# gercap/gr-ofdm_tools

Hardware: AMD Instinct MI355X
Metric: IQ Msamples/s Welch-PSD (4096-pt, 50% ovlp) (higher is better)
Workload: dtype f32; 1 GPU; C2: 2^28-sample complex64 stream, 4096-pt Hann Welch, 50% overlap, detrend constant, density; nfft=4096, noverlap=2048, window=hann, samples_per_gpu=268435456, segments_per_gpu=131071, parallelism=single GPU

## Files before the change

gr-ofdm_tools_amd/csrc/fft4096.hip.h:

```cpp
#pragma once
#include "fft_lds.hip.h"
#include "oth_internal.h"
#include "pinned_load.hip.h"
#include "twiddle16.hip.h"

static_assert(oth::kPilotProbes == 8, "load_pilot() (fft_lds.hip.h) adds eight probe means");

namespace oth {
namespace {

constexpr int T4 = 256;
constexpr int RS = 272;
constexpr int LDS_X = 16 * RS;
constexpr int LDS_RED = 16;
constexpr size_t LDS_BYTES = (LDS_X + LDS_RED) * sizeof(float2);

constexpr float C1 = 0.92387953251128674f;
constexpr float S1 = 0.38268343236508977f;
constexpr float RH = 0.70710678118654752f;

__device__ __forceinline__ float2 mul_w1(float2 a) { return make_float2(fmaf(a.x, C1, a.y * S1), fmaf(a.y, C1, -a.x * S1)); }
__device__ __forceinline__ float2 mul_w2(float2 a) { return make_float2((a.x + a.y) * RH, (a.y - a.x) * RH); }
__device__ __forceinline__ float2 mul_w3(float2 a) { return make_float2(fmaf(a.x, S1, a.y * C1), fmaf(a.y, S1, -a.x * C1)); }
__device__ __forceinline__ float2 mul_w4(float2 a) { return make_float2(a.y, -a.x); }
__device__ __forceinline__ float2 mul_w6(float2 a) { return make_float2((a.y - a.x) * RH, -(a.x + a.y) * RH); }
__device__ __forceinline__ float2 mul_w9(float2 a) { return make_float2(-fmaf(a.x, C1, a.y * S1), fmaf(a.x, S1, -a.y * C1)); }

constexpr float T1 = 0.41421356237309503f;

__device__ __forceinline__ void dft4_tail(float2 t0, float2 t1, float2 p1, float2 p3, float S, float2 &a0, float2 &a1,
                                          float2 &a2, float2 &a3) {
    const float2 q = cadd(p1, p3), r = csub(p1, p3);
    a0 = make_float2(fmaf(S, q.x, t0.x), fmaf(S, q.y, t0.y));
    a2 = make_float2(fmaf(-S, q.x, t0.x), fmaf(-S, q.y, t0.y));
    a1 = make_float2(fmaf(S, r.y, t1.x), fmaf(-S, r.x, t1.y));
    a3 = make_float2(fmaf(-S, r.y, t1.x), fmaf(S, r.x, t1.y));
}
template <bool PLAIN = false>
__device__ __forceinline__ void dft16_layer2(float2 (&v)[16]) {
  if constexpr (PLAIN) {
    v[5] = mul_w1(v[5]);
    v[9] = mul_w2(v[9]);
    v[13] = mul_w3(v[13]);
    v[6] = mul_w2(v[6]);
    v[10] = mul_w4(v[10]);
    v[14] = mul_w6(v[14]);
    v[7] = mul_w3(v[7]);
    v[11] = mul_w6(v[11]);
    v[15] = mul_w9(v[15]);
#pragma unroll
    for (int kl = 0; kl < 4; ++kl) dft4<false>(v[4 * kl], v[4 * kl + 1], v[4 * kl + 2], v[4 * kl + 3]);
  } else {
    dft4<false>(v[0], v[1], v[2], v[3]);
    {
        const float2 u1 = v[5], u2 = v[6], u3 = v[7];
        const float2 p1 = make_float2(fmaf(T1, u1.y, u1.x), fmaf(-T1, u1.x, u1.y));
        const float2 p2 = make_float2(u2.x + u2.y, u2.y - u2.x);
        const float2 p3 = make_float2(fmaf(T1, u3.x, u3.y), fmaf(T1, u3.y, -u3.x));
        const float2 t0 = make_float2(fmaf(RH, p2.x, v[4].x), fmaf(RH, p2.y, v[4].y));
        const float2 t1 = make_float2(fmaf(-RH, p2.x, v[4].x), fmaf(-RH, p2.y, v[4].y));
        dft4_tail(t0, t1, p1, p3, C1, v[4], v[5], v[6], v[7]);
    }
    {
        const float2 u1 = v[9], u2 = v[10], u3 = v[11];
        const float2 p1 = make_float2(u1.x + u1.y, u1.y - u1.x);
        const float2 p3 = make_float2(u3.y - u3.x, -u3.x - u3.y);
        const float2 t0 = make_float2(v[8].x + u2.y, v[8].y - u2.x);
        const float2 t1 = make_float2(v[8].x - u2.y, v[8].y + u2.x);
        dft4_tail(t0, t1, p1, p3, RH, v[8], v[9], v[10], v[11]);
    }
    {
        const float2 u1 = v[13], u2 = v[14], u3 = v[15];
        const float2 p1 = make_float2(fmaf(T1, u1.x, u1.y), fmaf(T1, u1.y, -u1.x));
        const float2 p2 = make_float2(u2.y - u2.x, -u2.x - u2.y);
        const float2 p3 = make_float2(fmaf(-T1, u3.y, -u3.x), fmaf(T1, u3.x, -u3.y));
        const float2 t0 = make_float2(fmaf(RH, p2.x, v[12].x), fmaf(RH, p2.y, v[12].y));
        const float2 t1 = make_float2(fmaf(-RH, p2.x, v[12].x), fmaf(-RH, p2.y, v[12].y));
        dft4_tail(t0, t1, p1, p3, C1, v[12], v[13], v[14], v[15]);
    }
  }
}

template <bool PLAIN = false>
__device__ __forceinline__ void dft16(float2 (&v)[16]) {
#pragma unroll
    for (int a0 = 0; a0 < 4; ++a0) dft4<false>(v[a0], v[a0 + 4], v[a0 + 8], v[a0 + 12]);
    dft16_layer2<PLAIN>(v);
}

template <bool PLAIN = false>
__device__ __forceinline__ void dft8(float2 (&v)[8]) {
    dft4<false>(v[0], v[2], v[4], v[6]);
    dft4<false>(v[1], v[3], v[5], v[7]);
    const float2 e0 = v[0], e1 = v[2], e2 = v[4], e3 = v[6];
    const float2 o0 = v[1], o2 = mul_w4(v[5]);
    if constexpr (PLAIN) {
        const float2 o1 = mul_w2(v[3]), o3 = mul_w6(v[7]);
        v[0] = cadd(e0, o0);
        v[4] = csub(e0, o0);
        v[1] = cadd(e1, o1);
        v[5] = csub(e1, o1);
        v[2] = cadd(e2, o2);
        v[6] = csub(e2, o2);
        v[3] = cadd(e3, o3);
        v[7] = csub(e3, o3);
        return;
    }
    const float2 p1 = make_float2(v[3].x + v[3].y, v[3].y - v[3].x);
    const float2 p3 = make_float2(v[7].y - v[7].x, -v[7].x - v[7].y);
    v[0] = cadd(e0, o0);
    v[4] = csub(e0, o0);
    v[1] = make_float2(fmaf(RH, p1.x, e1.x), fmaf(RH, p1.y, e1.y));
    v[5] = make_float2(fmaf(-RH, p1.x, e1.x), fmaf(-RH, p1.y, e1.y));
    v[2] = cadd(e2, o2);
    v[6] = csub(e2, o2);
    v[3] = make_float2(fmaf(RH, p3.x, e3.x), fmaf(RH, p3.y, e3.y));
    v[7] = make_float2(fmaf(-RH, p3.x, e3.x), fmaf(-RH, p3.y, e3.y));
}

typedef float lds_f4 __attribute__((ext_vector_type(4)));
template <bool WORD, bool SUMS> struct LdsCtl {
    const int *word_at;
    const float2 *sums_at;
    int word;
    lds_f4 s[2];
};
struct LdsNoMid {
    __device__ __forceinline__ void operator()() const {}
};

template <int STRIDE, class F, class M = LdsNoMid, bool WORD = false, bool SUMS = false>
__device__ __forceinline__ void dft16_from_lds(float2 (&v)[16], const float2 *base, F issued, M mid = M(),
                                               LdsCtl<WORD, SUMS> *ctl = nullptr) {
    const unsigned addr = (unsigned)(unsigned long long)base;
    double r[16];
    if constexpr (WORD) asm volatile("ds_read_b32 %0, %1" : "=v"(ctl->word) : "v"((unsigned)(unsigned long long)ctl->word_at));
    if constexpr (SUMS) {
        const unsigned sa = (unsigned)(unsigned long long)ctl->sums_at;
        asm volatile("ds_read_b128 %0, %1" : "=v"(ctl->s[0]) : "v"(sa));
        asm volatile("ds_read_b128 %0, %1 offset:16" : "=v"(ctl->s[1]) : "v"(sa));
    }
#define OTH_LDS_READ(i) asm volatile("ds_read_b64 %0, %1 offset:%2" : "=v"(r[i]) : "v"(addr), "n"(8 * STRIDE * (i)))
    OTH_LDS_READ(0); OTH_LDS_READ(4); OTH_LDS_READ(8); OTH_LDS_READ(12);
    OTH_LDS_READ(1); OTH_LDS_READ(5); OTH_LDS_READ(9); OTH_LDS_READ(13);
    OTH_LDS_READ(2); OTH_LDS_READ(6); OTH_LDS_READ(10); OTH_LDS_READ(14);
    OTH_LDS_READ(3); OTH_LDS_READ(7); OTH_LDS_READ(11); OTH_LDS_READ(15);
#undef OTH_LDS_READ
    issued();
#define OTH_LDS_WAIT(n, a, dep) \
    asm volatile("s_waitcnt lgkmcnt(" #n ")" : "+v"(r[a]), "+v"(r[a + 4]), "+v"(r[a + 8]), "+v"(r[a + 12]), "+v"(dep))
#pragma unroll
    for (int a0 = 0; a0 < 4; ++a0) {
        if (a0 == 0) {
            asm volatile("s_waitcnt lgkmcnt(12)" : "+v"(r[0]), "+v"(r[4]), "+v"(r[8]), "+v"(r[12]));
            if constexpr (SUMS) asm volatile("" : "+v"(ctl->s[0]), "+v"(ctl->s[1]));
        } else if (a0 == 1) OTH_LDS_WAIT(8, 1, v[0].x);
        else if (a0 == 2) OTH_LDS_WAIT(4, 2, v[1].x);
        else OTH_LDS_WAIT(0, 3, v[2].x);
#pragma unroll
        for (int j = 0; j < 4; ++j) v[a0 + 4 * j] = __builtin_bit_cast(float2, r[a0 + 4 * j]);
        dft4<false>(v[a0], v[a0 + 4], v[a0 + 8], v[a0 + 12]);
    }
#undef OTH_LDS_WAIT
    if constexpr (WORD) asm volatile("" : "+v"(ctl->word), "+v"(v[3].x), "+v"(v[15].y));
    mid();
    dft16_layer2(v);
}

__device__ __forceinline__ float2 load_once(const float2 *p) {
    typedef float f2 __attribute__((ext_vector_type(2)));
    const f2 r = __builtin_nontemporal_load(reinterpret_cast<const f2 *>(p));
    return make_float2(r.x, r.y);
}

__device__ __forceinline__ long long chunk_count(const WelchArgs &p) {
    const long long rest = p.nseg - p.nbig * p.chunk;
    return p.nbig + (rest + p.tail_chunk - 1) / p.tail_chunk;
}
__device__ __forceinline__ void chunk_range(const WelchArgs &p, long long c, long long &sb, long long &se) {
    if (c < p.nbig) {
        sb = c * p.chunk;
        se = sb + p.chunk;
    } else {
        sb = p.nbig * p.chunk + (c - p.nbig) * p.tail_chunk;
        se = sb + p.tail_chunk < p.nseg ? sb + p.tail_chunk : p.nseg;
    }
}

template <class I> __device__ __forceinline__ I chunk_count_of(I nseg, I nbig, int chunk, int tail_chunk) {
    const I rest = nseg - nbig * chunk;
    return nbig + (rest + tail_chunk - 1) / tail_chunk;
}
template <class I> __device__ __forceinline__ void chunk_range_of(I nseg, I nbig, int chunk, int tail_chunk, I c, I &sb, I &se) {
    if (c < nbig) {
        sb = c * chunk;
        se = sb + chunk;
    } else {
        sb = nbig * chunk + (c - nbig) * tail_chunk;
        se = sb + tail_chunk < nseg ? sb + tail_chunk : nseg;
    }
}

__device__ __forceinline__ void prio_latency() { __builtin_amdgcn_s_setprio(2); }
__device__ __forceinline__ void prio_compute() { __builtin_amdgcn_s_setprio(0); }

__device__ __forceinline__ void lds_barrier() { asm volatile("s_waitcnt lgkmcnt(0)\n\ts_barrier" ::: "memory"); }

__host__ __device__ constexpr int pow16_slot(int k) { return k - 5 - (k >> 2) + 1; }
template <int STRIDE, int NM>
__device__ __forceinline__ void scatter_pow16_stored(const float2 (&v)[16], float2 *out, float2 p1, float2 p2, float2 p3, float2 p4,
                                                     float2 p8, float2 p12, const float2 (&pm)[NM]) {
    float2 wj[4], wi[4];
    wj[1] = p1, wj[2] = p2, wj[3] = p3;
    wi[1] = p4, wi[2] = p8, wi[3] = p12;
#pragma unroll
    for (int i = 1; i < 4; ++i)
        if (pow16_slot(4 * i + 3) >= NM) asm volatile("" : "+v"(wi[i].x), "+v"(wi[i].y));
    out[0] = v[0];
#pragma unroll
    for (int k = 1; k < 16; ++k) {
        const int i = k >> 2, j = k & 3;
        float2 w;
        if (i == 0) w = wj[j];
        else if (j == 0) w = wi[i];
        else if (pow16_slot(k) < NM) w = pm[pow16_slot(k) < NM ? pow16_slot(k) : 0];
        else w = cmul(wi[i], wj[j]);
        out[STRIDE * k] = cmul(v[r16(k)], w);
    }
}

__device__ __forceinline__ void wave_lds_sync() {
    __builtin_amdgcn_fence(__ATOMIC_RELEASE, "wavefront");
    __builtin_amdgcn_wave_barrier();
    __builtin_amdgcn_fence(__ATOMIC_ACQUIRE, "wavefront");
}

template <int CTRL> __device__ __forceinline__ float dpp_add(float v) {
    const int x = __builtin_amdgcn_update_dpp(0, __float_as_int(v), CTRL, 0xF, 0xF, true);
    return v + __int_as_float(x);
}

__device__ __forceinline__ float wave_total(float v) {
    v = dpp_add<0xB1>(v);
    v = dpp_add<0x4E>(v);
    v = dpp_add<0x141>(v);
    v = dpp_add<0x140>(v);
    const int i = __float_as_int(v);
    return __int_as_float(__builtin_amdgcn_readlane(i, 0)) + __int_as_float(__builtin_amdgcn_readlane(i, 16)) +
           __int_as_float(__builtin_amdgcn_readlane(i, 32)) + __int_as_float(__builtin_amdgcn_readlane(i, 48));
}

__device__ __forceinline__ float wave_total_lane63(float v) {
    v = dpp_add<0xB1>(v);
    v = dpp_add<0x4E>(v);
    v = dpp_add<0x141>(v);
    v = dpp_add<0x140>(v);
    asm("s_nop 1\n\tv_add_f32_dpp %0, %0, %0 row_bcast:15 row_mask:0xa bank_mask:0xf" : "+v"(v));
    asm("s_nop 1\n\tv_add_f32_dpp %0, %0, %0 row_bcast:31 row_mask:0xc bank_mask:0xf" : "+v"(v));
    return v;
}

struct PilotProbes {
    float2 v[kPilotProbes];
};
__device__ __forceinline__ PilotProbes inline_pilot_load(const float2 *xb, long long nseg, int step, int t) {
    PilotProbes r;
#pragma unroll
    for (int k = 0; k < kPilotProbes; ++k) {
        const long long seg = ((nseg - 1) * k) / (kPilotProbes - 1);
        const float2 *src = xb + (size_t)__builtin_amdgcn_readfirstlane((int)seg) * (size_t)step + 512 * k;
        r.v[k] = src[(unsigned)t];
    }
    return r;
}
__device__ __forceinline__ void inline_pilot_store(const PilotProbes &r, int t, float2 *slot) {
#pragma unroll
    for (int k = 0; k < kPilotProbes; ++k) {
        const float2 s = make_float2(wave_total_lane63(r.v[k].x), wave_total_lane63(r.v[k].y));
        if ((t & 63) == 63) slot[4 * k + (t >> 6)] = s;
    }
}
__device__ __forceinline__ float2 inline_pilot_value(const float2 *slot) {
    float2 q[kPilotProbes];
#pragma unroll
    for (int k = 0; k < kPilotProbes; ++k) {
        const float2 a = cadd(slot[4 * k], slot[4 * k + 1]), b = cadd(slot[4 * k + 2], slot[4 * k + 3]);
        q[k] = make_float2((a.x + b.x) * (1.0f / 256.0f), (a.y + b.y) * (1.0f / 256.0f));
    }
    return pilot_of_probes(q);
}


}
}
```

gr-ofdm_tools_amd/csrc/welch4096ws.hip:

```cpp

#include <type_traits>
#include "fft4096.hip.h"
#include "launch.h"

namespace oth {
namespace {

constexpr int TWS = 512;
constexpr int WS_RED = 32;
constexpr int WS_CTRL = 16;
constexpr size_t WS_WIN_BYTES = 256 * 2 * sizeof(float4);
constexpr size_t WS_LDS_BYTES = (2 * LDS_X + WS_RED) * sizeof(float2) + WS_CTRL * sizeof(int) + WS_WIN_BYTES;

constexpr int WS_PAL = 2, WS_PAC = 0, WS_PAS = WS_PAL, WS_PBL = 2;
constexpr int WS_PBC = 1;

enum { ITEM_STOP = 0, ITEM_DATA = 1, ITEM_BUBBLE = 2 };

#ifndef OTH_WS_COMPL_POWERS
#define OTH_WS_COMPL_POWERS 13
#endif
constexpr int WS_COMPL_POWERS = OTH_WS_COMPL_POWERS;

template <bool DETREND, bool PILOT, bool COMPL>
__device__ __forceinline__ void welch4096ws_body(const WelchArgs &p) {
    static_assert(DETREND || !PILOT, "the pilot belongs to the detrend");
    extern __shared__ __attribute__((aligned(16))) unsigned char smem[];
    float2 *img = reinterpret_cast<float2 *>(smem);
    float2 *red = img + 2 * LDS_X;
    int *ctrl = reinterpret_cast<int *>(red + WS_RED);

    const int tid = threadIdx.x;
    const bool producer = tid < 256;
    const int t = tid & 255;
    const int hi = t >> 4, lo = t & 15;
    const int wave = t >> 6;
    const int wg = blockIdx.x, W = p.wg_per_stream, stream = blockIdx.y;
    const float2 *xb = p.x + (size_t)stream * p.stream_stride;
    const int sched = p.sched;
    const long long nchunks = sched ? chunk_count(p) : 1;

    const int w1 = hi * 17 + lo, r1 = hi * RS + lo, w2 = hi * RS + lo, r2 = hi * RS + lo * 17;

    if (producer) {
        float win[COMPL ? 1 : 8];
        float4 *wl = reinterpret_cast<float4 *>(ctrl + WS_CTRL) + t;
        constexpr int WROW = COMPL ? 0 : 8;
        if constexpr (!COMPL) {
#pragma unroll
            for (int a = 0; a < 8; ++a) win[a] = p.win[256 * a + t];
        }
        wl[0] = make_float4(p.win[256 * WROW + t], p.win[256 * (WROW + 1) + t], p.win[256 * (WROW + 2) + t], p.win[256 * (WROW + 3) + t]);
        wl[256] = make_float4(p.win[256 * (WROW + 4) + t], p.win[256 * (WROW + 5) + t], p.win[256 * (WROW + 6) + t],
                              p.win[256 * (WROW + 7) + t]);
        const float2 b1 = p.tw[t], b2 = p.tw[2 * t], b3 = p.tw[3 * t], b4 = p.tw[4 * t], b8 = p.tw[8 * t],
                     b12 = p.tw[(12 * t) & 4095];
        float2 bm[WS_COMPL_POWERS - 6 > 0 && COMPL ? WS_COMPL_POWERS - 6 : 1];
        if constexpr (COMPL) {
#pragma unroll
            for (int k = 0; k < WS_COMPL_POWERS - 6; ++k) bm[k] = p.tw[((5 + k + k / 3) * t) & 4095];
        }
        float2 kw[8], nxt[8];
        float2 prev_new = make_float2(0.f, 0.f);
        float2 pv = make_float2(0.f, 0.f);
        if (PILOT && !p.pilot_inline) pv = load_pilot(p.pilot, stream);
        int it = 0;
        unsigned ticket = 0;
        using std::false_type;
        using std::true_type;
        using mid = std::integral_constant<int, 0>;
        using head = std::integral_constant<int, 1>;
        using none = std::integral_constant<int, 2>;

        auto uni = [](int v) { return __builtin_amdgcn_readfirstlane(v); };
        auto load_chunk_head = [&](int first_seg) {
            const float2 *xs = xb + (size_t)uni(first_seg) * 2048;
#pragma unroll
            for (int j = 0; j < 4; ++j) {
                const float2 *xj = xs + 512 * j;
                kw[2 * j] = *(xj + (unsigned)t);
                kw[2 * j + 1] = *(xj + ((unsigned)t + 256u));
            }
#pragma unroll
            for (int j = 0; j < 4; ++j) {
                const float2 *xj = xs + 2048 + 512 * j;
                nxt[2 * j] = load_once(xj + (unsigned)t);
                nxt[2 * j + 1] = load_once(xj + ((unsigned)t + 256u));
            }
        };
        auto step_end = [&](int item) {
            if (t == 0) ctrl[it & 1] = item;
            lds_barrier();
            ++it;
        };
        auto item = [&](auto first_, auto mode_, int s, int nsb, bool publish) {
            constexpr bool FIRST = decltype(first_)::value;
            constexpr int MODE = decltype(mode_)::value;
            const int q = it & 1;
            float2 *lx = img + q * LDS_X;
            if constexpr (COMPL) asm volatile("; item %0 %1" ::"n"((int)FIRST), "n"(MODE));
            __builtin_amdgcn_s_setprio(WS_PAL);
            float2 v[16];
            float2 sumf = make_float2(0.f, 0.f), sum = make_float2(0.f, 0.f);
            const float4 wa = wl[0], wb = wl[256];
            const float wh[8] = {wa.x, wa.y, wa.z, wa.w, wb.x, wb.y, wb.z, wb.w};
            if (FIRST) {
#pragma unroll
                for (int a = 0; a < 8; ++a) {
                    if (PILOT) kw[a] = csub(kw[a], pv);
                    sumf = cadd(sumf, kw[a]);
                    if constexpr (!COMPL) kw[a] = make_float2(kw[a].x * win[a], kw[a].y * win[a]);
                }
            }
#pragma unroll
            for (int a = 0; a < 8; ++a) {
                const float2 r = PILOT ? csub(nxt[a], pv) : nxt[a];
                if constexpr (COMPL) {
                    v[a] = make_float2(kw[a].x * wh[a], kw[a].y * wh[a]);
                    v[8 + a] = make_float2(fmaf(-r.x, wh[a], r.x), fmaf(-r.y, wh[a], r.y));
                    if (MODE == 0) kw[a] = r;
                } else {
                    v[a] = kw[a];
                    v[8 + a] = make_float2(r.x * wh[a], r.y * wh[a]);
                    if (MODE == 0) kw[a] = make_float2(r.x * win[a], r.y * win[a]);
                }
                sum = (COMPL && a == 0) ? r : cadd(sum, r);
            }
            if (sched == 2 && t == 0) {
                if (FIRST) ticket = atomicAdd(p.queue + stream, 1u);
                if (publish) ctrl[4] = (int)ticket;
            }
            const float2 *xn = xb + (size_t)uni(s + 2) * 2048;
            auto load_next = [&]() {
#pragma unroll
                for (int j = 0; j < 4; ++j) {
                    const float2 *xj = xn + 512 * j;
                    nxt[2 * j] = load_once(xj + (unsigned)t);
                    nxt[2 * j + 1] = load_once(xj + ((unsigned)t + 256u));
                }
            };
            if (MODE == 0) {
                load_next();
            } else if (MODE == 1) {
                load_chunk_head(nsb);
            }
            if (DETREND) {
                sum.x = wave_total_lane63(sum.x);
                sum.y = wave_total_lane63(sum.y);
                float2 other = prev_new;
                if (FIRST) other = make_float2(wave_total_lane63(sumf.x), wave_total_lane63(sumf.y));
                if ((t & 63) == 63) red[q * 8 + wave] = cadd(sum, other);
                prev_new = sum;
            }
            __builtin_amdgcn_s_setprio(WS_PAC);
            dft16(v);
            __builtin_amdgcn_s_setprio(WS_PAS);
            if constexpr (COMPL) scatter_pow16_stored<RS>(v, lx + w1, b1, b2, b3, b4, b8, b12, bm);
            else scatter_pow16_six<RS>(v, lx + w1, Pow6{b1, b2, b3, b4, b8, b12});
            step_end(ITEM_DATA);
        };

        int cur = 0, sb = 0, se = 0;
        auto range = [&](int c, int &b, int &e) {
            long long lb, le;
            chunk_range(p, c, lb, le);
            b = uni((int)lb);
            e = uni((int)le);
        };
        auto open_chunk = [&](int c) -> bool {
            cur = c;
            if (sched) {
                if (cur >= nchunks) return false;
                range(cur, sb, se);
                return true;
            }
            sb = uni((int)((p.nseg * wg) / W));
            se = uni((int)((p.nseg * (wg + 1)) / W));
            return sb < se;
        };
        bool have = open_chunk(sched ? wg : 0);
        if (have) load_chunk_head(sb);
        if (PILOT && p.pilot_inline) {
            const bool own = sched == 0 && have;
            const PilotProbes probes = inline_pilot_load(own ? xb + (size_t)sb * 2048 : xb, own ? (long long)(se - sb) : p.nseg, 2048, t);
            inline_pilot_store(probes, t, img + LDS_X);
            lds_barrier();
            pv = inline_pilot_value(img + LDS_X);
        }
        while (have) {
            const int n = se - sb;
            int ncur = 0;
            if (n >= 2) {
                item(true_type{}, mid{}, sb, 0, n == 2);
                int s = sb + 1;
                if (s < se - 1) item(false_type{}, mid{}, s++, 0, true);
                for (; s + 1 < se - 1; s += 2) {
                    item(false_type{}, mid{}, s, 0, false);
                    item(false_type{}, mid{}, s + 1, 0, false);
                }
                if (s < se - 1) item(false_type{}, mid{}, s, 0, false);
                ncur = (sched == 1) ? cur + W : W + uni(ctrl[4]);
                int nsb = 0, nse = 0;
                const bool have_next = sched && ncur < nchunks;
                if (have_next) {
                    range(ncur, nsb, nse);
                    item(false_type{}, head{}, se - 1, nsb, false);
                    cur = ncur;
                    sb = nsb;
                    se = nse;
                    continue;
                }
                item(false_type{}, none{}, se - 1, 0, false);
                break;
            }
            item(true_type{}, none{}, sb, 0, true);
            if (sched == 0) break;
            if (sched == 2) {
                step_end(ITEM_BUBBLE);
                ncur = W + uni(ctrl[4]);
            } else {
                ncur = cur + W;
            }
            have = open_chunk(ncur);
            if (have) load_chunk_head(sb);
        }
        step_end(ITEM_STOP);
    } else {
        float2 tw2[16];
#pragma unroll
        for (int k = 1; k < 16; ++k) tw2[k] = p.tw[16 * lo * k];
        float4 fw = make_float4(0.f, 0.f, 0.f, 0.f);
        if (DETREND) fw = p.fd[t];
        float acc[16];
#pragma unroll
        for (int k = 0; k < 16; ++k) acc[k] = 0.f;
        float2 v[16];
        float2 mean = make_float2(0.f, 0.f);
        asm volatile("s_waitcnt vmcnt(0)"
                     : "+v"(tw2[1].x), "+v"(tw2[1].y), "+v"(tw2[2].x), "+v"(tw2[2].y), "+v"(tw2[3].x), "+v"(tw2[3].y), "+v"(tw2[4].x),
                       "+v"(tw2[4].y), "+v"(tw2[5].x), "+v"(tw2[5].y), "+v"(tw2[6].x), "+v"(tw2[6].y), "+v"(tw2[7].x), "+v"(tw2[7].y));
        asm volatile("" : "+v"(tw2[8].x), "+v"(tw2[8].y), "+v"(tw2[9].x), "+v"(tw2[9].y), "+v"(tw2[10].x), "+v"(tw2[10].y),
                          "+v"(tw2[11].x), "+v"(tw2[11].y), "+v"(tw2[12].x), "+v"(tw2[12].y), "+v"(tw2[13].x), "+v"(tw2[13].y));
        asm volatile("" : "+v"(tw2[14].x), "+v"(tw2[14].y), "+v"(tw2[15].x), "+v"(tw2[15].y), "+v"(fw.x), "+v"(fw.y), "+v"(fw.z),
                          "+v"(fw.w));
        int it = 0;
        auto pass2 = [&](int q) -> int {
            LdsCtl<true, DETREND> c;
            c.word_at = ctrl + q, c.sums_at = red + q * 8;
            dft16_from_lds<17>(v, img + q * LDS_X + r1, [] { __builtin_amdgcn_s_setprio(WS_PBC); }, LdsNoMid(), &c);
            if (DETREND) {
                const float2 h0 = make_float2(c.s[0].x, c.s[0].y), h1 = make_float2(c.s[0].z, c.s[0].w);
                const float2 h2 = make_float2(c.s[1].x, c.s[1].y), h3 = make_float2(c.s[1].z, c.s[1].w);
                const float2 tot = cadd(cadd(h0, h1), cadd(h2, h3));
                mean = make_float2(tot.x * (1.0f / 4096.0f), tot.y * (1.0f / 4096.0f));
            }
            return __builtin_amdgcn_readfirstlane(c.word);
        };
        auto next_item = [&]() -> int {
            __builtin_amdgcn_s_setprio(WS_PBL);
            lds_barrier();
            const int kind = pass2(it & 1);
            ++it;
            return kind;
        };
        auto idle_step = [&]() -> int {
            __builtin_amdgcn_s_setprio(WS_PBL);
            lds_barrier();
            const int kind = ctrl[it & 1];
            ++it;
            return kind;
        };
        if (PILOT && p.pilot_inline) lds_barrier();
        int item = next_item();
        while (item != ITEM_STOP) {
            float2 *lx = img + ((it & 1) ^ 1) * LDS_X;
            __builtin_amdgcn_s_setprio(WS_PBL);
            lx[w2] = v[r16(0)];
#pragma unroll
            for (int k1 = 1; k1 < 16; ++k1) lx[w2 + k1 * 17] = cmul(v[r16(k1)], tw2[k1]);
            wave_lds_sync();
            dft16_from_lds<1>(v, lx + r2, [] { __builtin_amdgcn_s_setprio(WS_PBC); });
            if (DETREND) {
                v[r16(0)] = make_float2(v[r16(0)].x - (mean.x * fw.x - mean.y * fw.y),
                                        v[r16(0)].y - (mean.x * fw.y + mean.y * fw.x));
                v[r16(15)] = make_float2(v[r16(15)].x - (mean.x * fw.z - mean.y * fw.w),
                                         v[r16(15)].y - (mean.x * fw.w + mean.y * fw.z));
            }
#pragma unroll
            for (int k2 = 0; k2 < 16; ++k2) {
                const float2 X = v[r16(k2)];
                acc[k2] = fmaf(X.x, X.x, fmaf(X.y, X.y, acc[k2]));
            }
            asm volatile("" : "+v"(acc[0]), "+v"(acc[1]), "+v"(acc[2]), "+v"(acc[3]), "+v"(acc[4]), "+v"(acc[5]), "+v"(acc[6]),
                              "+v"(acc[7]));
            asm volatile("" : "+v"(acc[8]), "+v"(acc[9]), "+v"(acc[10]), "+v"(acc[11]), "+v"(acc[12]), "+v"(acc[13]),
                              "+v"(acc[14]), "+v"(acc[15]));
            item = next_item();
            if (__builtin_expect(item == ITEM_BUBBLE, 0)) {
                do item = idle_step(); while (item == ITEM_BUBBLE);
                if (item == ITEM_DATA) pass2((it & 1) ^ 1);
            }
        }
        float *dst = p.partial + ((size_t)stream * W + wg) * 4096;
#pragma unroll
        for (int k2 = 0; k2 < 16; ++k2) dst[256 * k2 + t] = acc[k2];
    }
}

template <bool DETREND, bool PILOT = false>
__global__ __launch_bounds__(TWS, 4) void welch4096ws_kernel(WelchArgs p) {
    welch4096ws_body<DETREND, PILOT, false>(p);
}
template <bool DETREND, bool PILOT = false>
__global__ __launch_bounds__(TWS, 4) void welch4096ws_compl_kernel(WelchArgs p) {
    welch4096ws_body<DETREND, PILOT, true>(p);
}

}

int tuned4096_blocks_per_cu_ws() { return resident_blocks<welch4096ws_kernel<true, false>>(TWS, WS_LDS_BYTES); }

hipError_t launch_welch_tuned4096_ws(const WelchArgs &a, hipStream_t s) {
    const dim3 grid(a.wg_per_stream, a.nstreams);
    const bool pilot = a.detrend && (a.pilot || a.pilot_inline);
    if (!a.compl_win) {
        if (pilot) return launch_lds<welch4096ws_kernel<true, true>>(grid, dim3(TWS), WS_LDS_BYTES, s, a);
        if (a.detrend) return launch_lds<welch4096ws_kernel<true, false>>(grid, dim3(TWS), WS_LDS_BYTES, s, a);
        return launch_lds<welch4096ws_kernel<false, false>>(grid, dim3(TWS), WS_LDS_BYTES, s, a);
    }
    if (pilot) return launch_lds<welch4096ws_compl_kernel<true, true>>(grid, dim3(TWS), WS_LDS_BYTES, s, a);
    if (a.detrend) return launch_lds<welch4096ws_compl_kernel<true, false>>(grid, dim3(TWS), WS_LDS_BYTES, s, a);
    return launch_lds<welch4096ws_compl_kernel<false, false>>(grid, dim3(TWS), WS_LDS_BYTES, s, a);
}

}
```

Measured before the change: 438,500 Msamples/s.

## Fuse pass-2 twiddles into radix-4 reads and interleave LDS stores with compute

The inter-pass twiddle multiply moves from the store side to the load side. It is folded into a new FMA-based twiddled radix-4 butterfly that runs as each group of LDS reads completes. The first-pass results are now written to LDS group by group through a callback inside the second DFT16 layer, instead of in a separate store loop after the transform. This aims to overlap LDS stores with arithmetic and cut multiply/add count and register pressure, but it depends on the reading lane's twiddles matching the data layout.

Result: no change. 442,300 Msamples/s (median of 6 runs) (+0.9%).

```diff
diff --git a/gr-ofdm_tools_amd/csrc/fft4096.hip.h b/gr-ofdm_tools_amd/csrc/fft4096.hip.h
--- a/gr-ofdm_tools_amd/csrc/fft4096.hip.h
+++ b/gr-ofdm_tools_amd/csrc/fft4096.hip.h
@@ -36,8 +36,11 @@
     a1 = make_float2(fmaf(S, r.y, t1.x), fmaf(-S, r.x, t1.y));
     a3 = make_float2(fmaf(-S, r.y, t1.x), fmaf(S, r.x, t1.y));
 }
-template <bool PLAIN = false>
-__device__ __forceinline__ void dft16_layer2(float2 (&v)[16]) {
+struct Dft16NoDone {
+    __device__ __forceinline__ void operator()(int) const {}
+};
+template <bool PLAIN = false, class D = Dft16NoDone>
+__device__ __forceinline__ void dft16_layer2(float2 (&v)[16], D done = D()) {
   if constexpr (PLAIN) {
     v[5] = mul_w1(v[5]);
     v[9] = mul_w2(v[9]);
@@ -49,9 +52,13 @@
     v[11] = mul_w6(v[11]);
     v[15] = mul_w9(v[15]);
 #pragma unroll
-    for (int kl = 0; kl < 4; ++kl) dft4<false>(v[4 * kl], v[4 * kl + 1], v[4 * kl + 2], v[4 * kl + 3]);
+    for (int kl = 0; kl < 4; ++kl) {
+        dft4<false>(v[4 * kl], v[4 * kl + 1], v[4 * kl + 2], v[4 * kl + 3]);
+        done(kl);
+    }
   } else {
     dft4<false>(v[0], v[1], v[2], v[3]);
+    done(0);
     {
         const float2 u1 = v[5], u2 = v[6], u3 = v[7];
         const float2 p1 = make_float2(fmaf(T1, u1.y, u1.x), fmaf(-T1, u1.x, u1.y));
@@ -60,6 +67,7 @@
         const float2 t0 = make_float2(fmaf(RH, p2.x, v[4].x), fmaf(RH, p2.y, v[4].y));
         const float2 t1 = make_float2(fmaf(-RH, p2.x, v[4].x), fmaf(-RH, p2.y, v[4].y));
         dft4_tail(t0, t1, p1, p3, C1, v[4], v[5], v[6], v[7]);
+        done(1);
     }
     {
         const float2 u1 = v[9], u2 = v[10], u3 = v[11];
@@ -68,6 +76,7 @@
         const float2 t0 = make_float2(v[8].x + u2.y, v[8].y - u2.x);
         const float2 t1 = make_float2(v[8].x - u2.y, v[8].y + u2.x);
         dft4_tail(t0, t1, p1, p3, RH, v[8], v[9], v[10], v[11]);
+        done(2);
     }
     {
         const float2 u1 = v[13], u2 = v[14], u3 = v[15];
@@ -77,6 +86,7 @@
         const float2 t0 = make_float2(fmaf(RH, p2.x, v[12].x), fmaf(RH, p2.y, v[12].y));
         const float2 t1 = make_float2(fmaf(-RH, p2.x, v[12].x), fmaf(-RH, p2.y, v[12].y));
         dft4_tail(t0, t1, p1, p3, C1, v[12], v[13], v[14], v[15]);
+        done(3);
     }
   }
 }
@@ -129,9 +139,23 @@
     __device__ __forceinline__ void operator()() const {}
 };
 
-template <int STRIDE, class F, class M = LdsNoMid, bool WORD = false, bool SUMS = false>
+__device__ __forceinline__ void dft4_twiddled(bool ONE, float2 &a0, float2 &a1, float2 &a2, float2 &a3, float2 w0, float2 w1,
+                                              float2 w2, float2 w3) {
+    const float2 p0 = ONE ? a0 : cmul(a0, w0), p1 = cmul(a1, w1);
+    const float2 A = make_float2(fmaf(a2.x, w2.x, fmaf(-a2.y, w2.y, p0.x)), fmaf(a2.x, w2.y, fmaf(a2.y, w2.x, p0.y)));
+    const float2 C = make_float2(fmaf(a3.x, w3.x, fmaf(-a3.y, w3.y, p1.x)), fmaf(a3.x, w3.y, fmaf(a3.y, w3.x, p1.y)));
+    const float2 B = make_float2(fmaf(2.0f, p0.x, -A.x), fmaf(2.0f, p0.y, -A.y));
+    const float2 D = make_float2(fmaf(2.0f, p1.x, -C.x), fmaf(2.0f, p1.y, -C.y));
+    a0 = cadd(A, C);
+    a2 = csub(A, C);
+    a1 = make_float2(B.x + D.y, B.y - D.x);
+    a3 = make_float2(B.x - D.y, B.y + D.x);
+}
+
+struct LdsNoTw {};
+template <int STRIDE, class F, class M = LdsNoMid, bool WORD = false, bool SUMS = false, class TW = LdsNoTw, class D = Dft16NoDone>
 __device__ __forceinline__ void dft16_from_lds(float2 (&v)[16], const float2 *base, F issued, M mid = M(),
-                                               LdsCtl<WORD, SUMS> *ctl = nullptr) {
+                                               LdsCtl<WORD, SUMS> *ctl = nullptr, TW tw = TW(), D done = D()) {
     const unsigned addr = (unsigned)(unsigned long long)base;
     double r[16];
     if constexpr (WORD) asm volatile("ds_read_b32 %0, %1" : "=v"(ctl->word) : "v"((unsigned)(unsigned long long)ctl->word_at));
@@ -159,12 +183,20 @@
         else OTH_LDS_WAIT(0, 3, v[2].x);
 #pragma unroll
         for (int j = 0; j < 4; ++j) v[a0 + 4 * j] = __builtin_bit_cast(float2, r[a0 + 4 * j]);
-        dft4<false>(v[a0], v[a0 + 4], v[a0 + 8], v[a0 + 12]);
+        if constexpr (!std::is_same<TW, LdsNoTw>::value)
+            dft4_twiddled(a0 == 0, v[a0], v[a0 + 4], v[a0 + 8], v[a0 + 12], a0 ? tw(a0) : make_float2(1.f, 0.f), tw(a0 + 4),
+                          tw(a0 + 8), tw(a0 + 12));
+        else dft4<false>(v[a0], v[a0 + 4], v[a0 + 8], v[a0 + 12]);
     }
 #undef OTH_LDS_WAIT
     if constexpr (WORD) asm volatile("" : "+v"(ctl->word), "+v"(v[3].x), "+v"(v[15].y));
     mid();
-    dft16_layer2(v);
+    dft16_layer2<false>(v, done);
+}
+template <int STRIDE, class TW, class F, class M = LdsNoMid, bool WORD = false, bool SUMS = false>
+__device__ __forceinline__ void dft16_twiddled_from_lds(float2 (&v)[16], const float2 *base, TW tw, F issued, M mid = M(),
+                                                        LdsCtl<WORD, SUMS> *ctl = nullptr) {
+    dft16_from_lds<STRIDE>(v, base, issued, mid, ctl, tw);
 }
 
 __device__ __forceinline__ float2 load_once(const float2 *p) {
diff --git a/gr-ofdm_tools_amd/csrc/welch4096ws.hip b/gr-ofdm_tools_amd/csrc/welch4096ws.hip
--- a/gr-ofdm_tools_amd/csrc/welch4096ws.hip
+++ b/gr-ofdm_tools_amd/csrc/welch4096ws.hip
@@ -247,7 +247,11 @@
         auto pass2 = [&](int q) -> int {
             LdsCtl<true, DETREND> c;
             c.word_at = ctrl + q, c.sums_at = red + q * 8;
-            dft16_from_lds<17>(v, img + q * LDS_X + r1, [] { __builtin_amdgcn_s_setprio(WS_PBC); }, LdsNoMid(), &c);
+            float2 *lx = img + q * LDS_X;
+            dft16_from_lds<17>(v, lx + r1, [] { __builtin_amdgcn_s_setprio(WS_PBC); }, LdsNoMid(), &c, LdsNoTw(), [&](int kl) {
+#pragma unroll
+                for (int m = 0; m < 4; ++m) lx[w2 + (kl + 4 * m) * 17] = v[4 * kl + m];
+            });
             if (DETREND) {
                 const float2 h0 = make_float2(c.s[0].x, c.s[0].y), h1 = make_float2(c.s[0].z, c.s[0].w);
                 const float2 h2 = make_float2(c.s[1].x, c.s[1].y), h3 = make_float2(c.s[1].z, c.s[1].w);
@@ -275,11 +279,8 @@
         while (item != ITEM_STOP) {
             float2 *lx = img + ((it & 1) ^ 1) * LDS_X;
             __builtin_amdgcn_s_setprio(WS_PBL);
-            lx[w2] = v[r16(0)];
-#pragma unroll
-            for (int k1 = 1; k1 < 16; ++k1) lx[w2 + k1 * 17] = cmul(v[r16(k1)], tw2[k1]);
             wave_lds_sync();
-            dft16_from_lds<1>(v, lx + r2, [] { __builtin_amdgcn_s_setprio(WS_PBC); });
+            dft16_twiddled_from_lds<1>(v, lx + r2, [&](int i) { return tw2[i]; }, [] { __builtin_amdgcn_s_setprio(WS_PBC); });
             if (DETREND) {
                 v[r16(0)] = make_float2(v[r16(0)].x - (mean.x * fw.x - mean.y * fw.y),
                                         v[r16(0)].y - (mean.x * fw.y + mean.y * fw.x));
```
